# drprojects/superpoint_transformer

Measured on AMD Instinct MI355X. Metric: Mpoints/s SPT fwd+bwd on S3DIS-scale NAG, higher is better.
Workload: dtype f32 (the reference's shipped matmul class - configs/train.yaml:60-61 `float32_matmul_precision: high` = TF32 / bf16x3 next to `precision: 32` - as bf16x3: matrix products on the bf16 pipe with split operands, attention and the backward of the fused layers and of the attention blocks' Linears hi*hi +

## Files before the change

include/spt_hip.h:

```cpp
#ifndef SPT_HIP_H
#define SPT_HIP_H

#include <stddef.h>
#include <stdint.h>

#ifdef __cplusplus
extern "C" {
#endif

typedef void* spt_stream_t;

enum spt_reduce_op {
  SPT_SUM = 0,
  SPT_MEAN = 1,
  SPT_MIN = 2,
  SPT_MAX = 3
};

typedef struct spt_gn_fwd_tables {
  const float* weight;
  const float* mean_scale;
  float eps;
  float* mean;
  float* rstd;
// ... 347 lines not shown
size_t spt_relabel_consecutive_workspace_bytes(int64_t n_range);
int spt_relabel_consecutive(const int64_t* values, const int64_t* gather, int64_t k,
                            int64_t n_range, int64_t* new_values, int64_t* uniques,
                            int64_t* count, void* ws, size_t ws_bytes, spt_stream_t stream);

int spt_horizontal_edge_features_f32(
    const int64_t* se, int64_t e, int64_t n, const float* edge_attr7, const float* pos,
    const float* normal, const float* log_length, const float* log_surface,
    const float* log_volume, const float* log_size, int add_self_loops,
    int64_t* edge_index_out, float* edge_attr_out, spt_stream_t stream);
int spt_vertical_edge_features_f32(
    const int64_t* super_index, int64_t n, const float* child_pos, const float* child_normal,
    const float* child_log_length, const float* child_log_surface, const float* child_log_volume,
    const float* child_log_size, const float* parent_pos, const float* parent_normal,
    const float* parent_log_length, const float* parent_log_surface,
    const float* parent_log_volume, const float* parent_log_size, float* v_edge_attr,
    spt_stream_t stream);
int spt_edge_affinity_features_f32(const float* x, int64_t n, int C, const int64_t* edge_a,
                                   const int64_t* edge_b, int64_t e, float* out,
                                   spt_stream_t stream);
int spt_edge_affinity_features_bwd_f32(const float* x, const float* gout, int64_t n, int C,
                                       const int64_t* edge_a, const int64_t* edge_b, int64_t e,
                                       float* gend, spt_stream_t stream);

int spt_skinny_linear_supported(int K, int N);
int spt_skinny_linear_f32(const float* x, int64_t rows, int K, const float* W, const float* bias,
                          int N, float* y, spt_stream_t stream);
int spt_skinny_linear_wt_f32(const float* x, int64_t rows, int K, const float* Wt, int N, float* y,
                             spt_stream_t stream);
int spt_skinny_pre_supported(int K, int N, int num_graphs);
int spt_skinny_linear_pre_f32(const float* x, int64_t rows, int K, const float* W, const float* bias,
                              int N, float* y, const float* pre_am, const float* pre_scale,
                              const float* pre_bias, const int64_t* batch, int num_graphs,
                              const float* residual, spt_stream_t stream);
int spt_skinny_dw_pre_f32(const float* gy, const float* x, int64_t rows, int N, int K, float* gw,
                          float* gb, const float* pre_am, const float* pre_scale,
                          const float* pre_bias, const int64_t* batch, int num_graphs, void* ws,
                          size_t ws_bytes, spt_stream_t stream);
int spt_skinny_use_split_bf16(int mode);
int spt_skinny_linear_pre_m_f32(const float* x, int64_t rows, int K, const float* W, const float* bias,
                                int N, float* y, const float* pre_am, const float* pre_scale,
                                const float* pre_bias, const int64_t* batch, int num_graphs,
                                const float* residual, int mode, spt_stream_t stream);
int spt_skinny_linear_wt_m_f32(const float* x, int64_t rows, int K, const float* Wt, int N, float* y,
                               int mode, spt_stream_t stream);
int spt_skinny_dw_pre_m_f32(const float* gy, const float* x, int64_t rows, int N, int K, float* gw,
                            float* gb, const float* pre_am, const float* pre_scale,
                            const float* pre_bias, const int64_t* batch, int num_graphs, int mode,
                            void* ws, size_t ws_bytes, spt_stream_t stream);
int spt_skinny_dw_supported(int K, int N);
size_t spt_skinny_dw_workspace_bytes(int K, int N);
int spt_skinny_dw_f32(const float* gy, const float* x, int64_t rows, int N, int K, float* gw,
                      float* gb, void* ws, size_t ws_bytes, spt_stream_t stream);
int spt_narrow_linear_bwd_supported(int K, int N);
size_t spt_narrow_linear_bwd_workspace_bytes(int K, int N);
int spt_narrow_linear_bwd_f32(const float* gy, const float* x, const float* W, int64_t rows, int N,
                              int K, float* gx, float* gw, float* gb, void* ws, size_t ws_bytes,
                              spt_stream_t stream);

int spt_graphnorm_tables_f32(const double* total, int num_graphs, int d, const float* weight,
                             const float* mean_scale, float eps, float* mean, float* rstd,
                             float* am, float* scale, spt_stream_t stream);
int spt_graphnorm_apply_f32(const float* x, const int64_t* batch, int64_t r, int d,
                            int num_graphs, const float* am, const float* scale,
                            const float* bias, float act_slope, float* y, spt_stream_t stream);
int spt_graphnorm_bwd_stats_f32(const float* x, const float* gy, const int64_t* batch, int64_t r,
                                int d, int num_graphs, const float* am, const float* scale,
                                const float* bias, float act_slope, double* total, void* ws,
                                size_t ws_bytes, spt_stream_t stream);
size_t spt_graphnorm_bwd_stats_sparse_workspace_bytes(int64_t num_seg, int d, int num_graphs);
int spt_graphnorm_bwd_stats_sparse_f32(const float* x, const float* gout, const int32_t* arg,
                                       const int64_t* seg_graph, const int64_t* graph_rows,
                                       int64_t num_seg, int64_t n, int d, int num_graphs,
                                       const float* am, const float* scale, const float* bias,
                                       float act_slope, double* total, void* ws,
                                       size_t ws_bytes, spt_stream_t stream);
int spt_graphnorm_bwd_stats_sparse_ex_f32(
    const void* x, int x_is_bf16, const float* gout, const int32_t* arg, const int64_t* seg_graph,
    const int64_t* graph_rows, int64_t num_seg, int64_t n, int d, int num_graphs,
    const float* am, const float* scale, const float* bias, float act_slope, double* total,
    void* ws, size_t ws_bytes, spt_stream_t stream);
int spt_graphnorm_bwd_stats_sparse_raw_f32(
    const float* raw, const float* gout, const int32_t* arg, const int64_t* seg_graph,
    const int64_t* graph_rows, int64_t num_seg, int64_t n, int d, int num_graphs,
    const float* am, const float* scale, const float* bias, float act_slope, double* total,
    void* ws, size_t ws_bytes, spt_stream_t stream);
int spt_graphnorm_bwd_tables_f32(const double* total, int num_graphs, int d, const float* weight,
                                 const float* mean_scale, const float* mean, const float* rstd,
                                 float* c1, float* c2, float* c3, float* gweight, float* gbias,
                                 float* gmean_scale, spt_stream_t stream);

int spt_fused_linear_supported(int K, int N);
int spt_fused_linear_use_split_bf16(int mode);
size_t spt_fused_linear_workspace_bytes(int K, int N);
int spt_fused_linear_fwd_f32(const float* x, int64_t r0, int64_t r1, int K, const float* W,
                             int N, const float* pre_am, const float* pre_scale,
                             const float* pre_bias, float pre_slope, float* h, double* total,
                             void* ws, size_t ws_bytes, spt_stream_t stream);
int spt_fused_linear_bwd_f32(const float* gy, const float* h, int64_t r0, int64_t r1, int N,
                             const float* am, const float* scale, const float* bias,
                             float slope, const float* c1, const float* c2, const float* c3,
                             const float* xprev, int K, const float* pre_am,
                             const float* pre_scale, const float* pre_bias, float pre_slope,
                             const float* W, float* gx, float* gW, int accumulate,
                             double* prev_total, void* ws, size_t ws_bytes, spt_stream_t stream);
int spt_fused_linear_pooled_supported(int K, int N);
// ... 146 lines not shown
```

superpoint_transformer_amd/_lib.py:

```python
import ctypes
import os

import torch

_HERE = os.path.dirname(os.path.abspath(__file__))
LIB_PATH = os.path.join(_HERE, "lib", "libspt_hip.so")

_c = ctypes
_i64 = _c.c_int64
_int = _c.c_int
_p = _c.c_void_p
_sz = _c.c_size_t
_f32 = _c.c_float
_f64 = _c.c_double

SIGNATURES = {
    "spt_version": (_int, []),
    "spt_last_error": (_c.c_char_p, []),
    "spt_csr_build_workspace_bytes": (_sz, [_i64, _i64]),
    "spt_csr_build": (_int, [_p, _i64, _i64, _p, _p, _p, _sz, _p]),
    "spt_csr_pos_seg": (_int, [_p, _i64, _i64, _p, _p]),
    "spt_csr_gather_i64_i32": (_int, [_p, _p, _i64, _p, _p]),
    "spt_segcsr_reduce_f32": (_int, [_int, _p, _p, _p, _i64, _i64, _int, _p, _p, _p]),
    "spt_segcsr_max_affine_f32": (_int, [_p, _p, _p, _i64, _i64, _int, _p, _p, _p, _f32, _p, _p, _p, _p]),
# ... 132 lines not shown
                                                     _int, _p, _p, _p, _f32, _p, _p, _p, _p, _int, _p, _p,
                                                     _p, _f32, _p, _p, _p, _p, _p, _p, _int, _p, _sz, _p, _p]),
    "spt_csr_check_i64": (_int, [_p, _p, _p, _i64, _i64, _int, _p, _p]),
    "spt_csr_adopt_i64": (_int, [_p, _p, _p, _i64, _i64, _p, _p, _p, _p]),
    "spt_fused_linear_pool_supported": (_int, [_int, _int, _int]),
    "spt_fused_linear_pool_gram_len": (_sz, [_int]),
    "spt_fused_linear_pool_workspace_bytes": (_sz, [_int, _int]),
    "spt_fused_linear_fwd_pool_runs_f32": (_int, [_p, _p, _p, _p, _p, _i64, _i64, _int, _p, _p, _p, _int,
                                                  _int, _p, _int, _p, _p, _p, _f32, _f32, _p, _p, _p,
                                                  _f32, _p, _p, _p, _p, _p, _p, _p, _p, _p, _p, _int, _p,
                                                  _sz, _p]),
    "spt_fused_linear_bwd_pool_runs_f32": (_int, [_p, _p, _p, _p, _p, _p, _i64, _int, _p, _p, _p, _int,
                                                  _int, _p, _p, _p, _f32, _p, _p, _p, _p, _int, _p, _p,
                                                  _p, _f32, _p, _p, _p, _p, _p, _p, _int, _p, _sz, _p]),
    "spt_fused_linear_fwd_f32": (_int, [_p, _i64, _i64, _int, _p, _int, _p, _p, _p, _f32, _p, _p,
                                        _p, _sz, _p]),
    "spt_fused_linear_bwd_f32": (_int, [_p, _p, _i64, _i64, _int, _p, _p, _p, _f32, _p, _p, _p,
                                        _p, _int, _p, _p, _p, _f32, _p, _p, _p, _int, _p, _p,
                                        _sz, _p]),
    "spt_unit_sphere_norm_f32": (_int, [_p, _p, _p, _p, _p, _p, _i64, _i64, _p, _p, _p, _p]),
    "spt_unit_sphere_assemble_f32": (_int, [_p, _p, _p, _p, _p, _p, _i64, _i64, _p, _int, _p, _p, _p, _p]),
    "spt_unit_sphere_workspace_bytes": (_sz, [_i64, _i64]),
    "spt_unit_sphere_norm_ws_f32": (_int, [_p, _p, _p, _p, _p, _p, _i64, _i64, _p, _p, _p, _p, _sz, _p]),
    "spt_unit_sphere_assemble_ws_f32": (_int, [_p, _p, _p, _p, _p, _p, _i64, _i64, _p, _int, _p, _p, _p,
                                               _p, _sz, _p]),
    "spt_sparse_sample_workspace_bytes": (_sz, [_i64, _i64]),
    "spt_sparse_sample": (_int, [_p, _i64, _i64, _p, _int, _int, _c.c_uint64, _p, _p, _p, _sz, _p]),
    "spt_segment_std_f32": (_int, [_p, _p, _p, _i64, _int, _p, _p]),
    "spt_segment_mean_orientation_f32": (_int, [_p, _p, _p, _i64, _p, _p]),
    "spt_cluster_graph_edges_workspace_bytes": (_sz, [_i64, _int]),
    "spt_cluster_graph_edges": (_int, [_p, _p, _p, _i64, _int, _f32, _int, _p, _p, _p, _p, _sz, _p]),
    "spt_skinny_linear_supported": (_int, [_int, _int]),
    "spt_narrow_linear_bwd_supported": (_int, [_int, _int]),
    "spt_narrow_linear_bwd_workspace_bytes": (_sz, [_int, _int]),
    "spt_narrow_linear_bwd_f32": (_int, [_p, _p, _p, _i64, _int, _int, _p, _p, _p, _p, _sz, _p]),
    "spt_cross_entropy_workspace_bytes": (_sz, [_i64]),
    "spt_cross_entropy_fwd_f32": (_int, [_p, _p, _i64, _int, _i64, _p, _p, _p, _p, _sz, _p]),
    "spt_cross_entropy_bwd_f32": (_int, [_p, _p, _p, _i64, _int, _i64, _p, _p, _p, _p]),
    "spt_hist_loss_fwd_f32": (_int, [_p, _p, _i64, _int, _int, _int, _i64, _p, _p, _p, _p, _p, _sz, _p]),
    "spt_hist_loss_bwd_f32": (_int, [_p, _p, _i64, _int, _int, _int, _i64, _p, _p, _p, _p, _p]),
    "spt_confusion_matrix_i64": (_int, [_p, _p, _i64, _int, _int, _p, _p]),
    "spt_skinny_dw_supported": (_int, [_int, _int]),
    "spt_skinny_dw_workspace_bytes": (_sz, [_int, _int]),
    "spt_skinny_dw_f32": (_int, [_p, _p, _i64, _int, _int, _p, _p, _p, _sz, _p]),
    "spt_skinny_linear_f32": (_int, [_p, _i64, _int, _p, _p, _int, _p, _p]),
    "spt_skinny_linear_wt_f32": (_int, [_p, _i64, _int, _p, _int, _p, _p]),
    "spt_skinny_pre_supported": (_int, [_int, _int, _int]),
    "spt_skinny_linear_pre_f32": (_int, [_p, _i64, _int, _p, _p, _int, _p, _p, _p, _p, _p, _int, _p, _p]),
    "spt_skinny_dw_pre_f32": (_int, [_p, _p, _i64, _int, _int, _p, _p, _p, _p, _p, _p, _int, _p, _sz, _p]),
    "spt_skinny_use_split_bf16": (_int, [_int]),
    "spt_skinny_linear_pre_m_f32": (_int, [_p, _i64, _int, _p, _p, _int, _p, _p, _p, _p, _p, _int, _p, _int, _p]),
    "spt_skinny_linear_wt_m_f32": (_int, [_p, _i64, _int, _p, _int, _p, _int, _p]),
    "spt_skinny_dw_pre_m_f32": (_int, [_p, _p, _i64, _int, _int, _p, _p, _p, _p, _p, _p, _int, _int, _p, _sz, _p]),
    "spt_index_inverse": (_int, [_p, _i64, _i64, _p, _p]),
    "spt_select_edges_workspace_bytes": (_sz, [_i64]),
    "spt_select_edges": (_int, [_p, _i64, _i64, _p, _i64, _p, _i64, _p, _p, _p, _sz, _p]),
    "spt_cluster_select_workspace_bytes": (_sz, [_i64, _i64, _i64]),
    "spt_cluster_select": (_int, [_p, _p, _i64, _p, _i64, _i64, _p, _p, _p, _p, _p, _p, _sz, _p]),
    "spt_relabel_consecutive_workspace_bytes": (_sz, [_i64]),
    "spt_relabel_consecutive": (_int, [_p, _p, _i64, _i64, _p, _p, _p, _p, _sz, _p]),
    "spt_radius_ball_workspace_bytes": (_sz, [_i64]),
    "spt_radius_ball_f32": (_int, [_p, _i64, _p, _f32, _int, _p, _i64, _p, _p, _p, _sz, _p]),
    "spt_cluster_pair_anchors_f32": (_int, [_p, _p, _p, _p, _p, _i64, _i64, _int, _int, _p, _p, _p]),
    "spt_adjacency_stats_workspace_bytes": (_sz, [_i64]),
    "spt_adjacency_stats": (_int, [_p, _p, _i64, _i64, _int, _p, _p, _p, _sz, _p]),
    "spt_adjacency_regression": (_int, [_p, _p, _p, _i64, _i64, _int, _f32, _f32, _p, _p, _sz, _p]),
    "spt_adjacency_count_workspace_bytes": (_sz, [_i64]),
    "spt_adjacency_count": (_int, [_p, _i64, _i64, _int, _p, _p, _p, _i64, _int, _p, _p, _p, _sz, _p]),
    "spt_adjacency_fill_workspace_bytes": (_sz, [_i64, _i64]),
    "spt_adjacency_fill": (_int, [_p, _p, _i64, _i64, _int, _f32, _f32, _p, _p, _p, _p, _i64, _int, _int,
                                  _p, _p, _i64, _p, _p, _p, _p, _sz, _p]),
    "spt_ground_bounds_workspace_bytes": (_sz, [_i64]),
    "spt_ground_bounds_f32": (_int, [_p, _i64, _f32, _p, _p, _sz, _p]),
    "spt_ground_cell_min_f32": (_int, [_p, _i64, _f32, _i64, _i64, _i64, _i64, _p, _p]),
    "spt_ground_trim_workspace_bytes": (_sz, [_i64]),
    "spt_ground_trim_f32": (_int, [_p, _i64, _p, _int, _f32, _p, _f32, _p, _i64, _p, _i64, _p, _p, _sz, _p]),
    "spt_ground_ransac_workspace_bytes": (_sz, [_int]),
    "spt_ground_ransac_f32": (_int, [_p, _i64, _p, _p, _i64, _p, _p, _int, _f64, _p, _p, _p, _sz, _p]),
    "spt_ground_elevation_f32": (_int, [_p, _i64, _p, _f32, _p, _p]),
    "spt_point_color_workspace_bytes": (_sz, [_i64]),
    "spt_point_color_f32": (_int, [_p, _int, _i64, _int, _p, _i64, _p, _i64, _p, _i64, _p, _sz, _p]),
    "spt_point_density_f32": (_int, [_p, _i64, _p, _i64, _i64, _int, _p, _p]),
}


class GnFwdTables(ctypes.Structure):
    _fields_ = [("weight", _p), ("mean_scale", _p), ("eps", _f32), ("mean", _p), ("rstd", _p),
                ("am", _p), ("scale", _p)]


class GnBwdTables(ctypes.Structure):
    _fields_ = [("weight", _p), ("mean_scale", _p), ("mean", _p), ("rstd", _p), ("c1", _p), ("c2", _p),
                ("c3", _p), ("gweight", _p), ("gbias", _p), ("gmean_scale", _p)]


def _load():
    if not os.path.exists(LIB_PATH):
        raise ImportError(
            f"{LIB_PATH} is missing: run `python -c 'import __graft_entry__ as g; "
            f"g.build()'` (hipcc --offload-arch=gfx950). There is no fallback path.")
    lib = ctypes.CDLL(LIB_PATH)
    for name, (res, args) in SIGNATURES.items():
        fn = getattr(lib, name)
        fn.restype = res
        fn.argtypes = args
    return lib
# ... 29 lines not shown
```

superpoint_transformer_amd/csrc/skinny_linear.hip:

```cpp
#include "common.hpp"

namespace spt {
namespace skinny {

typedef float f32x4 __attribute__((ext_vector_type(4)));
constexpr int TR = 16;
constexpr int WAVES = 4;
constexpr int SLAB = 64;

typedef __bf16 bf16x8 __attribute__((ext_vector_type(8)));
typedef __bf16 bf16x4 __attribute__((ext_vector_type(4)));
typedef short s16x4 __attribute__((ext_vector_type(4)));

__host__ __device__ constexpr int skinny_planes(int PR) { return PR == 6 ? 3 : (PR == 3 ? 2 : 1); }
template <int NPL>
__device__ __forceinline__ void split_planes(const float (&x)[8], bf16x8 (&p)[NPL]) {
#pragma unroll
  for (int i = 0; i < 8; ++i) {
    const __bf16 a = (__bf16)x[i];
    p[0][i] = a;
    if constexpr (NPL >= 2) {
      const float r1 = x[i] - (float)a;
      const __bf16 b = (__bf16)r1;
      p[1][i] = b;
// ... 455 lines not shown
  }
  float* pw = partial + (size_t)wave * ((size_t)N * KF + N);
#pragma unroll
  for (int nb = 0; nb < 4; ++nb) {
    float v = bsum[nb];
    v += __shfl_xor(v, 16, 64);
    v += __shfl_xor(v, 32, 64);
    if (g == 0 && k0 == 0) pw[(size_t)N * KF + n0 + 16 * nb + c] = v;
  }
#pragma unroll
  for (int nb = 0; nb < 4; ++nb)
#pragma unroll
    for (int kb = 0; kb < KB; ++kb)
#pragma unroll
      for (int r = 0; r < 4; ++r)
        if (k0 + 16 * kb + c < KF)
          pw[(size_t)(n0 + 16 * nb + 4 * g + r) * KF + k0 + 16 * kb + c] = C[nb][kb][r];
}

__global__ __launch_bounds__(1024) void sum_tables_kernel(const float* __restrict__ partial, int ntab,
                                                          int len, int split, float* __restrict__ out0,
                                                          float* __restrict__ out1) {
  __shared__ float sl[64][17];
  const int cl = threadIdx.x & 15;
  const int col = blockIdx.x * 16 + cl;
  const int slice = threadIdx.x >> 4;
  float acc = 0.f;
  if (col < len) {
    const int per = (ntab + 63) / 64;
    const int lo = slice * per, hi = (lo + per < ntab) ? lo + per : ntab;
    int k = lo;
    for (; k + 16 <= hi; k += 16) {
      float a[16];
#pragma unroll
      for (int j = 0; j < 16; ++j) a[j] = partial[(size_t)(k + j) * len + col];
#pragma unroll
      for (int j = 0; j < 16; ++j) acc += a[j];
    }
    for (; k + 4 <= hi; k += 4) {
      const float a0 = partial[(size_t)k * len + col], a1 = partial[(size_t)(k + 1) * len + col];
      const float a2 = partial[(size_t)(k + 2) * len + col], a3 = partial[(size_t)(k + 3) * len + col];
      acc += a0; acc += a1; acc += a2; acc += a3;
    }
    for (; k < hi; ++k) acc += partial[(size_t)k * len + col];
  }
  sl[slice][cl] = acc;
  __syncthreads();
  if (slice == 0 && col < len) {
    float t = 0.f;
#pragma unroll
    for (int k = 0; k < 64; ++k) t += sl[k][cl];
    if (col < split) out0[col] = t;
    else if (out1) out1[col - split] = t;
  }
}

template <int NMAX>
__global__ __launch_bounds__(256) void narrow_linear_bwd_kernel(
    const float* __restrict__ gy, const float* __restrict__ x, const float* __restrict__ W,
    int64_t rows, int N, float* __restrict__ gx, float* __restrict__ partial, int K) {
  constexpr int RT = 16;
  const int lane = (threadIdx.x & 63) + 64 * blockIdx.y;
  const int64_t wave = (int64_t)blockIdx.x * (blockDim.x >> 6) + (threadIdx.x >> 6);
  const int64_t nwaves = (int64_t)gridDim.x * (blockDim.x >> 6);
  float w[NMAX], aw[NMAX], ab[NMAX];
#pragma unroll
  for (int n = 0; n < NMAX; ++n) {
    w[n] = (n < N) ? W[(size_t)n * K + lane] : 0.f;
    aw[n] = ab[n] = 0.f;
  }
  const int64_t nsteps = (rows + RT - 1) / RT;
  for (int64_t t = wave; t < nsteps; t += nwaves) {
    const int64_t row0 = t * RT;
    const int cnt = (int)((rows - row0) < RT ? (rows - row0) : RT);
    float gt[4];
    const int wl = threadIdx.x & 63;
#pragma unroll
    for (int q = 0; q < 4; ++q) {
      const int e = q * 64 + wl;
      gt[q] = (e < cnt * N) ? gy[row0 * N + e] : 0.f;
    }
    float xr[RT];
#pragma unroll
    for (int r = 0; r < RT; ++r) xr[r] = (r < cnt) ? x[(row0 + r) * K + lane] : 0.f;
    if (N == NMAX) {
#pragma unroll
      for (int r = 0; r < RT; ++r) {
        float dx = 0.f;
#pragma unroll
        for (int n = 0; n < NMAX; ++n) {
          const int e = r * NMAX + n;
          const float gv = __builtin_bit_cast(
              float, __builtin_amdgcn_readlane(__builtin_bit_cast(int, gt[e >> 6]), e & 63));
          dx = fmaf(gv, w[n], dx);
          aw[n] = fmaf(gv, xr[r], aw[n]);
          ab[n] += gv;
        }
        if (gx && r < cnt) gx[(row0 + r) * K + lane] = dx;
      }
    } else {
      for (int r = 0; r < cnt; ++r) {
        float dx = 0.f;
        for (int n = 0; n < N; ++n) {
          const int e = r * N + n;
          const float src = (e >> 6) == 0 ? gt[0] : ((e >> 6) == 1 ? gt[1] : ((e >> 6) == 2 ? gt[2] : gt[3]));
          const float gv = __shfl(src, e & 63, 64);
// ... 207 lines not shown
  }
  switch (K) {
#define SPT_SKINNY_PL(K4, PR_)                                                                     \
  skinny_linear_kernel<K4, 4, false, false, PR_><<<grid, WAVES * 64, 0, stream>>>(                 \
      x, rows, W, bias, N, y, nullptr, nullptr, nullptr, nullptr, 1, nullptr, ldwt);
#define SPT_SKINNY_PLS(K4)                                                                         \
  if (pr == 6) { SPT_SKINNY_PL(K4, 6) } else if (pr == 3) { SPT_SKINNY_PL(K4, 3) }                 \
  else if (pr == 1) { SPT_SKINNY_PL(K4, 1) } else { SPT_SKINNY_PL(K4, 0) }
    case 32:  SPT_SKINNY_PLS(8) break;
    case 64:  SPT_SKINNY_PLS(16) break;
#undef SPT_SKINNY_PLS
#undef SPT_SKINNY_PL
    case 128: skinny_linear_kernel<32><<<grid, WAVES * 64, 0, stream>>>(x, rows, W, bias, N, y, nullptr, nullptr, nullptr, nullptr, 1, nullptr, ldwt); break;
    case 256: {
      int64_t b4 = ceil_div(tiles, (int64_t)4);
      const int64_t cap4 = (int64_t)256 / slabs > 1 ? (int64_t)256 / slabs : 1;
      if (b4 > cap4) b4 = cap4;
      skinny_linear_wlds_kernel<64, 4><<<dim3((unsigned)b4, (unsigned)slabs), 4 * 64, 0, stream>>>(
          x, rows, W, bias, N, y, ldwt);
      break;
    }
    case 260: {
      int64_t b4 = ceil_div(tiles, (int64_t)4);
      const int64_t cap4 = (int64_t)256 / slabs > 1 ? (int64_t)256 / slabs : 1;
      if (b4 > cap4) b4 = cap4;
      skinny_linear_wlds_kernel<65, 4><<<dim3((unsigned)b4, (unsigned)slabs), 4 * 64, 0, stream>>>(
          x, rows, W, bias, N, y, ldwt);
      break;
    }
    default: {
      int64_t b8 = ceil_div(tiles, WAVES_L);
      const int64_t cap8 = (int64_t)256 * (K == 192 ? 2 : 1) / slabs > 1 ? (int64_t)256 * (K == 192 ? 2 : 1) / slabs : 1;
      if (b8 > cap8) b8 = cap8;
      if (K == 132)
        skinny_linear_wlds_kernel<33><<<dim3((unsigned)b8, (unsigned)slabs), WAVES_L * 64, 0, stream>>>(
            x, rows, W, bias, N, y, ldwt);
      else
      {
        const dim3 g8((unsigned)b8, (unsigned)slabs);
        if (pr >= 3)
          skinny_linear_wlds_kernel<48, WAVES_L, 3><<<g8, WAVES_L * 64, 0, stream>>>(x, rows, W, bias, N, y, ldwt);
        else if (pr == 1)
          skinny_linear_wlds_kernel<48, WAVES_L, 1><<<g8, WAVES_L * 64, 0, stream>>>(x, rows, W, bias, N, y, ldwt);
        else
          skinny_linear_wlds_kernel<48><<<g8, WAVES_L * 64, 0, stream>>>(x, rows, W, bias, N, y, ldwt);
      }
      break;
    }
  }
  SPT_CHECK_LAUNCH();
  return 0;
}

constexpr int NARROW_BLOCKS = 256;

extern "C" int spt_narrow_linear_bwd_supported(int K, int N) { return (K == 64 || K == 128) && N >= 1 && N <= 16; }
extern "C" size_t spt_narrow_linear_bwd_workspace_bytes(int K, int N) {
  return (size_t)NARROW_BLOCKS * 4 * (16 * K + 16) * sizeof(float);
}
extern "C" int spt_narrow_linear_bwd_f32(const float* gy, const float* x, const float* W,
                                         int64_t rows, int N, int K, float* gx, float* gw,
                                         float* gb, void* ws, size_t ws_bytes,
                                         spt_stream_t stream_) {
  hipStream_t stream = (hipStream_t)stream_;
  SPT_CHECK_ARG(rows >= 0, "bad shape");
  SPT_CHECK_ARG(spt_narrow_linear_bwd_supported(K, N), "(K, N) not built");
  SPT_CHECK_ARG(W && gw && (rows == 0 || (gy && x)), "null pointer");
  SPT_CHECK_ARG(ws && ws_bytes >= spt_narrow_linear_bwd_workspace_bytes(K, N), "workspace too small");
  if (rows == 0) {
    hipMemsetAsync(gw, 0, (size_t)N * K * sizeof(float), stream);
    if (gb) hipMemsetAsync(gb, 0, (size_t)N * sizeof(float), stream);
    return 0;
  }
  int64_t bx = ceil_div(ceil_div(rows, (int64_t)16), (int64_t)4);
  if (bx > NARROW_BLOCKS) bx = NARROW_BLOCKS;
  float* partial = (float*)ws;
  int nmax;
  if (N == 13) {
    nmax = 13;
    narrow_linear_bwd_kernel<13><<<dim3((unsigned)bx, K / 64), 256, 0, stream>>>(gy, x, W, rows, N, gx, partial, K);
  } else {
    nmax = 16;
    narrow_linear_bwd_kernel<16><<<dim3((unsigned)bx, K / 64), 256, 0, stream>>>(gy, x, W, rows, N, gx, partial, K);
  }
  (void)nmax;
  sum_tables_kernel<<<(N * (K + 1) + 15) / 16, 1024, 0, stream>>>(partial, (int)bx * 4, N * (K + 1), N * K,
                                                                  gw, gb);
  SPT_CHECK_LAUNCH();
  return 0;
}
```

superpoint_transformer_amd/ops.py:

```python
import contextlib
import ctypes
import os

import torch

from . import _lib
from . import precision as _precision
from .csr import EdgeCSR, SegmentCSR, csr_of, edge_csr_of

_OPS = {"sum": 0, "add": 0, "mean": 1, "min": 2, "max": 3}

_TIMERS = {}
_TIMER_PREFIXES = []
_TIMER_CAP = 8192


def enable_timer(name, prefix=False):
    _TIMERS[name] = []
    if prefix and name not in _TIMER_PREFIXES:
        _TIMER_PREFIXES.append(name)


def timer_count(name):
    return len(_TIMERS.get(name) or [])
# ... 804 lines not shown
    if (g.is_cuda and g.dtype == torch.float32 and weight.dtype == torch.float32 and g.dim() == 2
            and g.shape[0] >= _SKINNY_MIN_ROWS and n_in % 4 == 0 and n_in >= 64
            and _lib.lib.spt_skinny_linear_supported(n_out, n_in)):
        g = g.contiguous()
        w = weight.detach().contiguous()
        rows = g.shape[0]
        y = torch.empty((rows, n_in), dtype=torch.float32, device=g.device)
        with torch.cuda.device(g.device):
            st = _lib.lib.spt_skinny_linear_wt_m_f32(_lib.ptr(g), rows, n_out, _lib.ptr(w), n_in,
                                                     _lib.ptr(y), int(mode), _lib.stream_ptr(g.device))
        _lib.check(st, "spt_skinny_linear_wt_m_f32")
        return y
    wt = weight.detach().t().contiguous()
    return _skinny_launch(g, wt, None, mode) if _skinny_ok(g, wt) else g @ weight


def _dw_batched(g, x):
    n = x.shape[0]
    nb = n // _DW_CHUNK
    main = nb * _DW_CHUNK
    gw = None
    if nb > 0:
        gm = g[:main].view(nb, _DW_CHUNK, g.shape[1])
        xm = x[:main].view(nb, _DW_CHUNK, x.shape[1])
        gw = torch.bmm(gm.transpose(1, 2), xm).sum(0)
    if main < n:
        tail = g[main:].t() @ x[main:]
        gw = tail if gw is None else gw + tail
    return gw


def _skinny_dw_ok(g, x):
    return (x.is_cuda and x.dtype == torch.float32 and g.dtype == torch.float32
            and x.shape[0] >= _SKINNY_MIN_ROWS
            and _lib.lib.spt_skinny_dw_supported(x.shape[1], g.shape[1]))


def _skinny_dw(g, x, want_bias=False, mode=-1):
    g, x = g.contiguous(), x.detach().contiguous()
    rows, k = x.shape
    n = g.shape[1]
    gw = torch.empty((n, k), dtype=torch.float32, device=x.device)
    gb = torch.empty(n, dtype=torch.float32, device=x.device) if want_bias else None
    nb = _lib.lib.spt_skinny_dw_workspace_bytes(k, n)
    ws = _workspace(nb, x.device)
    with torch.cuda.device(x.device):
        st = _lib.lib.spt_skinny_dw_pre_m_f32(_lib.ptr(g), _lib.ptr(x), rows, n, k, _lib.ptr(gw),
                                              _lib.ptr(gb), None, None, None, None, 1, int(mode),
                                              _lib.ptr(ws), ws.numel(), _lib.stream_ptr(x.device))
    _lib.check(st, "spt_skinny_dw_pre_m_f32")
    return (gw, gb) if want_bias else gw


class _TallLinear(torch.autograd.Function):

    @staticmethod
    def forward(ctx, x, weight, bias):
        ctx.save_for_backward(x, weight)
        ctx.has_bias = bias is not None
        ctx.smode = _precision.skinny_mode()
        if _skinny_ok(x, weight):
            return _skinny_launch(x.detach(), weight.detach(), None if bias is None else bias.detach(),
                                  ctx.smode)
        return torch.nn.functional.linear(x, weight, bias)

    @staticmethod
    def backward(ctx, g):
        x, weight = ctx.saved_tensors
        g = g.contiguous()
        if (x.is_cuda and x.dtype == torch.float32 and g.dtype == torch.float32
                and weight.dtype == torch.float32 and x.shape[0] >= _SKINNY_MIN_ROWS
                and _lib.lib.spt_narrow_linear_bwd_supported(x.shape[1], g.shape[1])):
            xc, wc = x.detach().contiguous(), weight.detach().contiguous()
            rows, k = xc.shape
            n = g.shape[1]
            dev = xc.device
            gx = torch.empty_like(xc) if ctx.needs_input_grad[0] else None
            gw = torch.empty((n, k), dtype=torch.float32, device=dev)
            gb = torch.empty(n, dtype=torch.float32, device=dev) if ctx.has_bias else None
            nb = _lib.lib.spt_narrow_linear_bwd_workspace_bytes(k, n)
            ws = _workspace(nb, dev)
            with torch.cuda.device(dev):
                st = _lib.lib.spt_narrow_linear_bwd_f32(
                    _lib.ptr(g), _lib.ptr(xc), _lib.ptr(wc), rows, n, k, _lib.ptr(gx),
                    _lib.ptr(gw), _lib.ptr(gb), _lib.ptr(ws), ws.numel(), _lib.stream_ptr(dev))
            _lib.check(st, "spt_narrow_linear_bwd_f32")
            return gx, gw, gb
        gx = None
        smode = getattr(ctx, "smode", -1)
        if ctx.needs_input_grad[0]:
            gx = _input_grad(g, weight, smode)
        gw = gb = None
        want_gb = ctx.has_bias and ctx.needs_input_grad[2]
        if ctx.needs_input_grad[1]:
            if _skinny_dw_ok(g, x):
                gw = _skinny_dw(g, x, want_gb, smode)
                if want_gb:
                    gw, gb = gw
            else:
                gw = _dw_batched(g, x) if x.shape[0] >= 4 * _DW_CHUNK else g.t() @ x
        if want_gb and gb is None:
            gb = g.sum(0)
        return gx, gw, gb


def linear(x, weight, bias=None):
    if x.dim() != 2 or not x.is_cuda or x.shape[0] < _SKINNY_MIN_ROWS:
        return torch.nn.functional.linear(x, weight, bias)
    return _TallLinear.apply(x, weight, bias)


class _ResidualLinear(torch.autograd.Function):

    @staticmethod
    def forward(ctx, x, weight, bias, residual):
        ctx.save_for_backward(x, weight)
        ctx.has_bias = bias is not None
        ctx.smode = _precision.skinny_mode()
        xd, wd = x.detach().contiguous(), weight.detach().contiguous()
        rows, k = xd.shape
        n = wd.shape[0]
        y = torch.empty((rows, n), dtype=torch.float32, device=xd.device)
        with torch.cuda.device(xd.device):
            st = _lib.lib.spt_skinny_linear_pre_m_f32(
                _lib.ptr(xd), rows, k, _lib.ptr(wd),
                _lib.ptr(None if bias is None else bias.detach().contiguous()), n, _lib.ptr(y),
                None, None, None, None, 1, _lib.ptr(residual.detach().contiguous()),
                ctx.smode, _lib.stream_ptr(xd.device))
        _lib.check(st, "spt_skinny_linear_pre_m_f32")
        return y

    @staticmethod
    def backward(ctx, g):
        gx, gw, gb = _TallLinear.backward(ctx, g)
        return gx, gw, gb, g


_FUSE_PRENORM = os.environ.get("SPT_FUSE_PRENORM", "1") != "0"


def fuse_prenorm(on=None):
    global _FUSE_PRENORM
    prev = _FUSE_PRENORM
    if on is not None:
        _FUSE_PRENORM = bool(on)
    return prev
# ... 11 lines not shown
            and linear_residual_ok(residual, weight)):
        return _ResidualLinear.apply(x, weight, bias, residual)
    return residual + linear(x, weight, bias)


class _NormLinear(torch.autograd.Function):

    @staticmethod
    def forward(ctx, x, batch, num_graphs, gn_w, gn_b, gn_a, eps, weight, bias):
        _lib.require_cuda(x)
        xd = x.detach().contiguous()
        rows, d = xd.shape
        dev = xd.device
        B = int(num_graphs)
        if batch is not None:
            batch = batch.contiguous()
            if batch.dtype != torch.int64:
                batch = batch.long()
        w, b, a = (t.detach().float().contiguous() for t in (gn_w, gn_b, gn_a))
        wd = weight.detach().contiguous()
        bd = None if bias is None else bias.detach().contiguous()
        n = wd.shape[0]
        mean, rstd, am, sc = (torch.empty((B, d), dtype=torch.float32, device=dev) for _ in range(4))
        y = torch.empty((rows, n), dtype=torch.float32, device=dev)
        nb = _lib.lib.spt_graphnorm_workspace_bytes(rows, d, B)
        ws = _workspace(nb, dev)
        with torch.cuda.device(dev):
            st = _lib.lib.spt_graphnorm_stats_f32(
                _lib.ptr(xd), _lib.ptr(batch), rows, d, B, _lib.ptr(w), _lib.ptr(a), float(eps),
                _lib.ptr(mean), _lib.ptr(rstd), _lib.ptr(am), _lib.ptr(sc), _lib.ptr(ws),
                ws.numel(), _lib.stream_ptr(dev))
            _lib.check(st, "spt_graphnorm_stats_f32")
            smode = _precision.skinny_mode()
            st = _lib.lib.spt_skinny_linear_pre_m_f32(
                _lib.ptr(xd), rows, d, _lib.ptr(wd), _lib.ptr(bd), n, _lib.ptr(y), _lib.ptr(am),
                _lib.ptr(sc), _lib.ptr(b), _lib.ptr(batch), B, None, smode, _lib.stream_ptr(dev))
        _lib.check(st, "spt_skinny_linear_pre_m_f32")
        ctx.save_for_backward(xd, batch, w, b, a, mean, rstd, am, sc, wd)
        ctx.meta = (B, bias is not None)
        ctx.smode = smode
        ctx.set_materialize_grads(False)
        return y, x

    @staticmethod
    def backward(ctx, gy, gres):
        xd, batch, w, b, a, mean, rstd, am, sc, wd = ctx.saved_tensors
        B, has_bias = ctx.meta
        if gy is None:
            return gres, None, None, None, None, None, None, None, None
        rows, d = xd.shape
        n = wd.shape[0]
        dev = xd.device
        gy = gy.contiguous()
        gxn = _input_grad(gy, wd, ctx.smode)
        gw = torch.empty((n, d), dtype=torch.float32, device=dev)
        gb = torch.empty(n, dtype=torch.float32, device=dev) if has_bias else None
        ws = _workspace(_lib.lib.spt_skinny_dw_workspace_bytes(d, n), dev)
        with torch.cuda.device(dev):
            st = _lib.lib.spt_skinny_dw_pre_m_f32(
                _lib.ptr(gy), _lib.ptr(xd), rows, n, d, _lib.ptr(gw), _lib.ptr(gb), _lib.ptr(am),
                _lib.ptr(sc), _lib.ptr(b), _lib.ptr(batch), B, ctx.smode, _lib.ptr(ws), ws.numel(),
                _lib.stream_ptr(dev))
        _lib.check(st, "spt_skinny_dw_pre_m_f32")
        gx = torch.empty_like(xd)
        g_w, g_b, g_a = (torch.empty(d, dtype=torch.float32, device=dev) for _ in range(3))
        if gres is not None:
            gres = gres.contiguous()
        ws = _workspace(_lib.lib.spt_graphnorm_workspace_bytes(rows, d, B), dev)
        with torch.cuda.device(dev):
            st = _lib.lib.spt_graphnorm_bwd_acc_f32(
                _lib.ptr(xd), _lib.ptr(gxn), _lib.ptr(batch), rows, d, B, _lib.ptr(w), _lib.ptr(b),
                _lib.ptr(a), _lib.ptr(mean), _lib.ptr(rstd), 1.0, _lib.ptr(gres), _lib.ptr(gx),
                _lib.ptr(g_w), _lib.ptr(g_b), _lib.ptr(g_a), _lib.ptr(ws), ws.numel(),
                _lib.stream_ptr(dev))
        _lib.check(st, "spt_graphnorm_bwd_acc_f32")
        return gx, None, None, g_w, g_b, g_a, None, gw, gb


def norm_linear_ok(x, batch, num_graphs, weight):
    if not _FUSE_PRENORM or (batch is not None and num_graphs is None):
        return False
    B = 1 if batch is None else int(num_graphs)
    return bool(x.dim() == 2 and x.is_cuda and x.dtype == torch.float32
                and weight.dtype == torch.float32 and x.shape[0] >= _SKINNY_MIN_ROWS
                and _lib.lib.spt_skinny_pre_supported(x.shape[1], weight.shape[0], B)
                and _lib.lib.spt_skinny_dw_supported(x.shape[1], weight.shape[0]))


_BCHK_ATTR = "_spt_batch_checked"


def _check_batch_ids(batch, B):
    if batch is None or _host_ptr(batch, B) is not None:
        return
    key = (batch._version, int(B), batch.data_ptr(), batch.numel())
    if getattr(batch, _BCHK_ATTR, None) == key:
        return
    if batch.numel():
        lo, hi = torch.aminmax(batch)
        if int(lo) < 0 or int(hi) >= int(B):
            raise ValueError(f"graph ids of `batch` must lie in [0, {int(B)}): found [{int(lo)}, {int(hi)}]")
    try:
        setattr(batch, _BCHK_ATTR, key)
    except Exception:
        pass


def norm_linear(x, batch, num_graphs, gn_weight, gn_bias, gn_mean_scale, eps, weight, bias):
    B = 1 if batch is None else int(num_graphs)
    _check_batch_ids(batch, B)
    return _NormLinear.apply(x, batch, B, gn_weight, gn_bias, gn_mean_scale, float(eps), weight, bias)


class _CrossEntropy(torch.autograd.Function):
    @staticmethod
    def forward(ctx, logits, target, ignore_index):
# ... 811 lines not shown
```

Baseline: 375.8.

## Fuse skinny linear backward input-grad and weight-grad into one bf16-split MFMA kernel

Measured after the change: 382.3, median of 6. 1.7% higher.

```diff
diff --git a/include/spt_hip.h b/include/spt_hip.h
--- a/include/spt_hip.h
+++ b/include/spt_hip.h
@@ -423,6 +423,14 @@
 size_t spt_skinny_dw_workspace_bytes(int K, int N);
 int spt_skinny_dw_f32(const float* gy, const float* x, int64_t rows, int N, int K, float* gw,
                       float* gb, void* ws, size_t ws_bytes, spt_stream_t stream);
+int spt_skinny_linear_bwd_supported(int K, int N, int num_graphs, int mode);
+size_t spt_skinny_linear_bwd_workspace_bytes(int K, int N);
+int spt_skinny_linear_bwd_m_f32(const float* gy, const float* x, const float* W, int64_t rows, int N,
+                                int K, float* gx, float* gw, float* gb, const float* pre_am,
+                                const float* pre_scale, const float* pre_bias, const int64_t* batch,
+                                int num_graphs, int mode, void* ws, size_t ws_bytes,
+                                spt_stream_t stream);
+int spt_skinny_bwd_fused(int on);
 int spt_narrow_linear_bwd_supported(int K, int N);
 size_t spt_narrow_linear_bwd_workspace_bytes(int K, int N);
 int spt_narrow_linear_bwd_f32(const float* gy, const float* x, const float* W, int64_t rows, int N,
diff --git a/superpoint_transformer_amd/_lib.py b/superpoint_transformer_amd/_lib.py
--- a/superpoint_transformer_amd/_lib.py
+++ b/superpoint_transformer_amd/_lib.py
@@ -208,6 +208,11 @@
     "spt_skinny_linear_pre_m_f32": (_int, [_p, _i64, _int, _p, _p, _int, _p, _p, _p, _p, _p, _int, _p, _int, _p]),
     "spt_skinny_linear_wt_m_f32": (_int, [_p, _i64, _int, _p, _int, _p, _int, _p]),
     "spt_skinny_dw_pre_m_f32": (_int, [_p, _p, _i64, _int, _int, _p, _p, _p, _p, _p, _p, _int, _int, _p, _sz, _p]),
+    "spt_skinny_linear_bwd_supported": (_int, [_int, _int, _int, _int]),
+    "spt_skinny_linear_bwd_workspace_bytes": (_sz, [_int, _int]),
+    "spt_skinny_linear_bwd_m_f32": (_int, [_p, _p, _p, _i64, _int, _int, _p, _p, _p, _p, _p, _p, _p, _int, _int,
+                                           _p, _sz, _p]),
+    "spt_skinny_bwd_fused": (_int, [_int]),
     "spt_index_inverse": (_int, [_p, _i64, _i64, _p, _p]),
     "spt_select_edges_workspace_bytes": (_sz, [_i64]),
     "spt_select_edges": (_int, [_p, _i64, _i64, _p, _i64, _p, _i64, _p, _p, _p, _sz, _p]),
diff --git a/superpoint_transformer_amd/csrc/skinny_linear.hip b/superpoint_transformer_amd/csrc/skinny_linear.hip
--- a/superpoint_transformer_amd/csrc/skinny_linear.hip
+++ b/superpoint_transformer_amd/csrc/skinny_linear.hip
@@ -531,6 +531,197 @@
     for (int k = 0; k < 64; ++k) t += sl[k][cl];
     if (col < split) out0[col] = t;
     else if (out1) out1[col - split] = t;
+  }
+}
+
+constexpr int BF_ROWS = 64;
+constexpr int BF_WAVES = 8;
+constexpr int BF_BLOCKS = 256;
+__host__ __device__ constexpr int bf_per_cu(int NN) { return NN == 64 ? 2 : 1; }
+typedef __attribute__((address_space(3))) bf16x4 lds_bf16x4;
+__device__ __forceinline__ bf16x8 read_tr_operand(const __bf16* at, int ld) {
+  const bf16x4 a = __builtin_amdgcn_ds_read_tr16_b64_v4bf16((lds_bf16x4*)at);
+  const bf16x4 b = __builtin_amdgcn_ds_read_tr16_b64_v4bf16((lds_bf16x4*)(at + 16 * ld));
+  return __builtin_shufflevector(a, b, 0, 1, 2, 3, 4, 5, 6, 7);
+}
+template <int NPL>
+__device__ __forceinline__ void split_planes4(const float4& v, bf16x4 (&p)[NPL]) {
+  const float x[4] = {v.x, v.y, v.z, v.w};
+#pragma unroll
+  for (int i = 0; i < 4; ++i) {
+    const __bf16 a = (__bf16)x[i];
+    p[0][i] = a;
+    if constexpr (NPL >= 2) p[1][i] = (__bf16)(x[i] - (float)a);
+  }
+}
+template <int NN, bool PRE, int PR>
+__global__ __launch_bounds__(BF_WAVES * 64, 2 * bf_per_cu(NN)) void skinny_bwd_fused_kernel(
+    const float* __restrict__ gy, const float* __restrict__ x, const float* __restrict__ W, int64_t rows,
+    float* __restrict__ gx, float* __restrict__ partial, const float* __restrict__ pam,
+    const float* __restrict__ psc, const float* __restrict__ pbs, const int64_t* __restrict__ batch,
+    int PB) {
+  constexpr int K = 64, NT = BF_WAVES * 64, LDG = NN + 16, LDX = K + 16, LDW = NN + 8;
+  constexpr int NPL = skinny_planes(PR), KS = NN / 32, NBW = NN / 64;
+  constexpr int VG = BF_ROWS * NN / 4 / NT, VX = BF_ROWS * K / 4 / NT;
+  static_assert(NN % 64 == 0 && (PR == 1 || PR == 3), "whole 64-column slabs, a bf16 mode");
+  static_assert(BF_ROWS * NN / 4 % NT == 0 && BF_ROWS * K / 4 % NT == 0, "whole float4 rounds");
+  constexpr int GPL = NPL == 1 ? 2 : NPL;
+  static_assert(GPL * BF_ROWS * LDG * 2 >= BF_ROWS * NN * 4, "the gb slots fit the gy planes");
+  __shared__ __attribute__((aligned(16))) __bf16 g_pl[GPL * BF_ROWS * LDG];
+  __shared__ __attribute__((aligned(16))) __bf16 x_pl[NPL * BF_ROWS * LDX];
+  __shared__ __attribute__((aligned(16))) __bf16 w_pl[NPL * K * LDW];
+  __shared__ __attribute__((aligned(16))) float ptab[PRE ? 2 * PRE_MAX + K : 4];
+  const int tid = threadIdx.x;
+  const int lane = tid & 63;
+  const int wid = __builtin_amdgcn_readfirstlane(tid >> 6);
+  const int g = lane >> 4, c = lane & 15;
+
+  for (int q = tid; q < K * (NN / 8); q += NT) {
+    const int k = q & (K - 1), n8 = q / K;
+    float wv[8];
+#pragma unroll
+    for (int j = 0; j < 8; ++j) wv[j] = W[(size_t)(8 * n8 + j) * K + k];
+    bf16x8 pl[NPL];
+    split_planes<NPL>(wv, pl);
+#pragma unroll
+    for (int p = 0; p < NPL; ++p) *reinterpret_cast<bf16x8*>(w_pl + p * K * LDW + k * LDW + 8 * n8) = pl[p];
+  }
+  if constexpr (PRE) {
+    for (int i = tid; i < PB * K; i += NT) {
+      ptab[i] = pam[i];
+      ptab[PRE_MAX + i] = psc[i];
+    }
+    for (int i = tid; i < K; i += NT) ptab[2 * PRE_MAX + i] = pbs[i];
+  }
+
+  const int rt = wid >> 1, nh = wid & 1;
+  const int kp = wid & 1, nb0 = (wid >> 1) * NBW;
+  f32x4 CW[NBW][2];
+#pragma unroll
+  for (int i = 0; i < NBW; ++i) CW[i][0] = CW[i][1] = (f32x4){0.f, 0.f, 0.f, 0.f};
+  float4 bs[VG];
+#pragma unroll
+  for (int v = 0; v < VG; ++v) bs[v] = make_float4(0.f, 0.f, 0.f, 0.f);
+
+  const int64_t ntiles = (rows + BF_ROWS - 1) / BF_ROWS;
+  float4 ng[VG], nx[VX];
+  int xg[VX];
+  auto fetch = [&](int64_t t) {
+    const int64_t gbase = t * BF_ROWS * (int64_t)NN, glim = rows * (int64_t)NN;
+#pragma unroll
+    for (int v = 0; v < VG; ++v) {
+      const int64_t e = gbase + (int64_t)(v * NT + tid) * 4;
+      ng[v] = (e < glim) ? *reinterpret_cast<const float4*>(gy + e) : make_float4(0.f, 0.f, 0.f, 0.f);
+    }
+#pragma unroll
+    for (int v = 0; v < VX; ++v) {
+      const int q = v * NT + tid;
+      const int64_t row = t * BF_ROWS + q / (K / 4);
+      nx[v] = (row < rows) ? *reinterpret_cast<const float4*>(x + row * K + (q & (K / 4 - 1)) * 4)
+                           : make_float4(0.f, 0.f, 0.f, 0.f);
+      if constexpr (PRE) xg[v] = (row < rows) ? (batch ? (int)batch[row] : 0) : -1;
+    }
+  };
+  if ((int64_t)blockIdx.x < ntiles) fetch(blockIdx.x);
+  for (int64_t t = blockIdx.x; t < ntiles; t += gridDim.x) {
+    __syncthreads();
+#pragma unroll
+    for (int v = 0; v < VG; ++v) {
+      const int q4 = (v * NT + tid) * 4, rr = q4 / NN, col = q4 - rr * NN;
+      bs[v].x += ng[v].x; bs[v].y += ng[v].y; bs[v].z += ng[v].z; bs[v].w += ng[v].w;
+      bf16x4 pl[NPL];
+      split_planes4<NPL>(ng[v], pl);
+#pragma unroll
+      for (int p = 0; p < NPL; ++p) *reinterpret_cast<bf16x4*>(g_pl + p * BF_ROWS * LDG + rr * LDG + col) = pl[p];
+    }
+#pragma unroll
+    for (int v = 0; v < VX; ++v) {
+      const int q = v * NT + tid, rr = q / (K / 4), ch = q & (K / 4 - 1);
+      float4 w = nx[v];
+      if constexpr (PRE) {
+        if (xg[v] >= 0) {
+          const float4 a = *reinterpret_cast<const float4*>(ptab + xg[v] * K + ch * 4);
+          const float4 sc4 = *reinterpret_cast<const float4*>(ptab + PRE_MAX + xg[v] * K + ch * 4);
+          const float4 b4 = *reinterpret_cast<const float4*>(ptab + 2 * PRE_MAX + ch * 4);
+          w.x = fmaf(w.x - a.x, sc4.x, b4.x); w.y = fmaf(w.y - a.y, sc4.y, b4.y);
+          w.z = fmaf(w.z - a.z, sc4.z, b4.z); w.w = fmaf(w.w - a.w, sc4.w, b4.w);
+        }
+      }
+      bf16x4 pl[NPL];
+      split_planes4<NPL>(w, pl);
+#pragma unroll
+      for (int p = 0; p < NPL; ++p) *reinterpret_cast<bf16x4*>(x_pl + p * BF_ROWS * LDX + rr * LDX + ch * 4) = pl[p];
+    }
+    __syncthreads();
+    if (t + gridDim.x < ntiles) fetch(t + gridDim.x);
+
+    {
+      f32x4 C[2] = {(f32x4){0.f, 0.f, 0.f, 0.f}, (f32x4){0.f, 0.f, 0.f, 0.f}};
+      const __bf16* al = g_pl + (16 * rt + c) * LDG + 8 * g;
+#pragma unroll
+      for (int ks = 0; ks < KS; ++ks) {
+        bf16x8 Ap[NPL];
+#pragma unroll
+        for (int p = 0; p < NPL; ++p) Ap[p] = *reinterpret_cast<const bf16x8*>(al + p * BF_ROWS * LDG + 32 * ks);
+#pragma unroll
+        for (int i = 0; i < 2; ++i) {
+          bf16x8 Bp[NPL];
+#pragma unroll
+          for (int p = 0; p < NPL; ++p)
+            Bp[p] = *reinterpret_cast<const bf16x8*>(w_pl + p * K * LDW + (16 * (2 * nh + i) + c) * LDW +
+                                                     32 * ks + 8 * g);
+          C[i] = mfma_planes<PR>(Ap, Bp, C[i]);
+        }
+      }
+#pragma unroll
+      for (int r = 0; r < 4; ++r) {
+        const int64_t row = t * BF_ROWS + 16 * rt + 4 * g + r;
+        if (row < rows) {
+#pragma unroll
+          for (int i = 0; i < 2; ++i)
+            __builtin_nontemporal_store(C[i][r], gx + row * K + 16 * (2 * nh + i) + c);
+        }
+      }
+    }
+
+#pragma unroll
+    for (int s = 0; s < BF_ROWS / 32; ++s) {
+      const int r0 = 32 * s + 4 * g + ((lane >> 2) & 3), c0 = 4 * (lane & 3);
+      bf16x8 Ap[NBW][NPL];
+#pragma unroll
+      for (int i = 0; i < NBW; ++i)
+#pragma unroll
+        for (int p = 0; p < NPL; ++p)
+          Ap[i][p] = read_tr_operand(g_pl + p * BF_ROWS * LDG + r0 * LDG + 16 * (nb0 + i) + c0, LDG);
+#pragma unroll
+      for (int kk = 0; kk < 2; ++kk) {
+        bf16x8 Bp[NPL];
+#pragma unroll
+        for (int p = 0; p < NPL; ++p)
+          Bp[p] = read_tr_operand(x_pl + p * BF_ROWS * LDX + r0 * LDX + 16 * (2 * kp + kk) + c0, LDX);
+#pragma unroll
+        for (int i = 0; i < NBW; ++i) CW[i][kk] = mfma_planes<PR>(Ap[i], Bp, CW[i][kk]);
+      }
+    }
+  }
+
+  float* pw = partial + (size_t)blockIdx.x * ((size_t)NN * K + NN);
+#pragma unroll
+  for (int i = 0; i < NBW; ++i)
+#pragma unroll
+    for (int kk = 0; kk < 2; ++kk)
+#pragma unroll
+      for (int r = 0; r < 4; ++r)
+        pw[(size_t)(16 * (nb0 + i) + 4 * g + r) * K + 16 * (2 * kp + kk) + c] = CW[i][kk][r];
+  __syncthreads();
+  float* slots = reinterpret_cast<float*>(g_pl);
+#pragma unroll
+  for (int v = 0; v < VG; ++v) *reinterpret_cast<float4*>(slots + (v * NT + tid) * 4) = bs[v];
+  __syncthreads();
+  if (tid < NN) {
+    float v = 0.f;
+    for (int rr = 0; rr < BF_ROWS; ++rr) v += slots[rr * NN + tid];
+    pw[(size_t)NN * K + tid] = v;
   }
 }
 
@@ -844,6 +1035,57 @@
   return 0;
 }
 
+static std::atomic<int> g_bwd_fused{[] { const char* e = getenv("SPT_SKINNY_BWD_FUSED"); return (e && atoi(e) == 0) ? 0 : 1; }()};
+extern "C" int spt_skinny_bwd_fused(int on) {
+  const int prev = g_bwd_fused;
+  if (on >= 0) g_bwd_fused = on ? 1 : 0;
+  return prev;
+}
+extern "C" int spt_skinny_linear_bwd_supported(int K, int N, int num_graphs, int mode) {
+  return K == 64 && (N == 64 || N == 192) && skinny_pr_bwd(mode) != 0 && num_graphs >= 1 &&
+         num_graphs * K <= PRE_MAX;
+}
+extern "C" size_t spt_skinny_linear_bwd_workspace_bytes(int K, int N) {
+  return (size_t)BF_BLOCKS * bf_per_cu(N) * N * (K + 1) * sizeof(float);
+}
+extern "C" int spt_skinny_linear_bwd_m_f32(const float* gy, const float* x, const float* W, int64_t rows,
+                                           int N, int K, float* gx, float* gw, float* gb,
+                                           const float* pre_am, const float* pre_scale,
+                                           const float* pre_bias, const int64_t* batch, int num_graphs,
+                                           int mode, void* ws, size_t ws_bytes, spt_stream_t stream_) {
+  const int pr = skinny_pr_bwd(mode);
+  hipStream_t stream = (hipStream_t)stream_;
+  SPT_CHECK_ARG(rows >= 0, "bad shape");
+  const bool pre = pre_am != nullptr;
+  SPT_CHECK_ARG(spt_skinny_linear_bwd_supported(K, N, pre ? num_graphs : 1, mode),
+                "(K, N) not built, the f32-exact mode or num_graphs * K too large");
+  SPT_CHECK_ARG(!pre || (pre_scale && pre_bias), "pre-normalisation: incomplete tables");
+  SPT_CHECK_ARG(gw && (rows == 0 || (gy && x && W && gx)), "null pointer");
+  SPT_CHECK_ARG(ws && ws_bytes >= spt_skinny_linear_bwd_workspace_bytes(K, N), "workspace too small");
+  if (rows == 0) {
+    hipMemsetAsync(gw, 0, (size_t)N * K * sizeof(float), stream);
+    if (gb) hipMemsetAsync(gb, 0, (size_t)N * sizeof(float), stream);
+    return 0;
+  }
+  int64_t bx = ceil_div(rows, (int64_t)BF_ROWS);
+  if (bx > BF_BLOCKS * bf_per_cu(N)) bx = BF_BLOCKS * bf_per_cu(N);
+  float* partial = (float*)ws;
+#define SPT_BF(NN_, PRE_, PR_)                                                                      \
+  skinny_bwd_fused_kernel<NN_, PRE_, PR_><<<(unsigned)bx, BF_WAVES * 64, 0, stream>>>(               \
+      gy, x, W, rows, gx, partial, pre_am, pre_scale, pre_bias, batch, num_graphs);
+#define SPT_BFS(NN_, PRE_) if (pr == 3) { SPT_BF(NN_, PRE_, 3) } else { SPT_BF(NN_, PRE_, 1) }
+  if (N == 192) {
+    if (pre) { SPT_BFS(192, true) } else { SPT_BFS(192, false) }
+  } else {
+    if (pre) { SPT_BFS(64, true) } else { SPT_BFS(64, false) }
+  }
+#undef SPT_BFS
+#undef SPT_BF
+  sum_tables_kernel<<<(N * (K + 1) + 15) / 16, 1024, 0, stream>>>(partial, (int)bx, N * (K + 1), N * K, gw, gb);
+  SPT_CHECK_LAUNCH();
+  return 0;
+}
+
 constexpr int NARROW_BLOCKS = 256;
 
 extern "C" int spt_narrow_linear_bwd_supported(int K, int N) { return (K == 64 || K == 128) && N >= 1 && N <= 16; }
diff --git a/superpoint_transformer_amd/ops.py b/superpoint_transformer_amd/ops.py
--- a/superpoint_transformer_amd/ops.py
+++ b/superpoint_transformer_amd/ops.py
@@ -880,6 +880,45 @@
     return (gw, gb) if want_bias else gw
 
 
+_BWD_ROUTE = {"fused": 0, "split": 0}
+
+
+def skinny_bwd_fused(on=None):
+    return bool(_lib.lib.spt_skinny_bwd_fused(-1 if on is None else int(bool(on))))
+
+
+def skinny_bwd_route_counts():
+    return dict(_BWD_ROUTE)
+
+
+def _skinny_bwd_ok(g, x, weight, num_graphs, mode):
+    return bool(x.is_cuda and x.dtype == torch.float32 and g.dtype == torch.float32
+                and weight.dtype == torch.float32 and x.dim() == 2 and x.shape[0] >= _SKINNY_MIN_ROWS
+                and _lib.lib.spt_skinny_bwd_fused(-1)
+                and _lib.lib.spt_skinny_linear_bwd_supported(x.shape[1], g.shape[1], int(num_graphs),
+                                                             int(mode)))
+
+
+def _skinny_bwd(g, x, weight, want_bias, mode, pre=None):
+    g, x, w = g.contiguous(), x.detach().contiguous(), weight.detach().contiguous()
+    rows, k = x.shape
+    n = g.shape[1]
+    dev = x.device
+    gx = torch.empty((rows, k), dtype=torch.float32, device=dev)
+    gw = torch.empty((n, k), dtype=torch.float32, device=dev)
+    gb = torch.empty(n, dtype=torch.float32, device=dev) if want_bias else None
+    am, sc, pb, batch, B = pre if pre is not None else (None, None, None, None, 1)
+    ws = _workspace(_lib.lib.spt_skinny_linear_bwd_workspace_bytes(k, n), dev)
+    with torch.cuda.device(dev):
+        st = _lib.lib.spt_skinny_linear_bwd_m_f32(
+            _lib.ptr(g), _lib.ptr(x), _lib.ptr(w), rows, n, k, _lib.ptr(gx), _lib.ptr(gw), _lib.ptr(gb),
+            _lib.ptr(am), _lib.ptr(sc), _lib.ptr(pb), _lib.ptr(batch), int(B), int(mode), _lib.ptr(ws),
+            ws.numel(), _lib.stream_ptr(dev))
+    _lib.check(st, "spt_skinny_linear_bwd_m_f32")
+    _BWD_ROUTE["fused"] += 1
+    return gx, gw, gb
+
+
 class _TallLinear(torch.autograd.Function):
 
     @staticmethod
@@ -916,10 +955,13 @@
             return gx, gw, gb
         gx = None
         smode = getattr(ctx, "smode", -1)
+        want_gb = ctx.has_bias and ctx.needs_input_grad[2]
+        if ctx.needs_input_grad[0] and ctx.needs_input_grad[1] and _skinny_bwd_ok(g, x, weight, 1, smode):
+            return _skinny_bwd(g, x, weight, want_gb, smode)
+        _BWD_ROUTE["split"] += 1
         if ctx.needs_input_grad[0]:
             gx = _input_grad(g, weight, smode)
         gw = gb = None
-        want_gb = ctx.has_bias and ctx.needs_input_grad[2]
         if ctx.needs_input_grad[1]:
             if _skinny_dw_ok(g, x):
                 gw = _skinny_dw(g, x, want_gb, smode)
@@ -1037,16 +1079,20 @@
         n = wd.shape[0]
         dev = xd.device
         gy = gy.contiguous()
-        gxn = _input_grad(gy, wd, ctx.smode)
-        gw = torch.empty((n, d), dtype=torch.float32, device=dev)
-        gb = torch.empty(n, dtype=torch.float32, device=dev) if has_bias else None
-        ws = _workspace(_lib.lib.spt_skinny_dw_workspace_bytes(d, n), dev)
-        with torch.cuda.device(dev):
-            st = _lib.lib.spt_skinny_dw_pre_m_f32(
-                _lib.ptr(gy), _lib.ptr(xd), rows, n, d, _lib.ptr(gw), _lib.ptr(gb), _lib.ptr(am),
-                _lib.ptr(sc), _lib.ptr(b), _lib.ptr(batch), B, ctx.smode, _lib.ptr(ws), ws.numel(),
-                _lib.stream_ptr(dev))
-        _lib.check(st, "spt_skinny_dw_pre_m_f32")
+        if ctx.needs_input_grad[7] and _skinny_bwd_ok(gy, xd, wd, B, ctx.smode):
+            gxn, gw, gb = _skinny_bwd(gy, xd, wd, has_bias, ctx.smode, (am, sc, b, batch, B))
+        else:
+            _BWD_ROUTE["split"] += 1
+            gxn = _input_grad(gy, wd, ctx.smode)
+            gw = torch.empty((n, d), dtype=torch.float32, device=dev)
+            gb = torch.empty(n, dtype=torch.float32, device=dev) if has_bias else None
+            ws = _workspace(_lib.lib.spt_skinny_dw_workspace_bytes(d, n), dev)
+            with torch.cuda.device(dev):
+                st = _lib.lib.spt_skinny_dw_pre_m_f32(
+                    _lib.ptr(gy), _lib.ptr(xd), rows, n, d, _lib.ptr(gw), _lib.ptr(gb), _lib.ptr(am),
+                    _lib.ptr(sc), _lib.ptr(b), _lib.ptr(batch), B, ctx.smode, _lib.ptr(ws), ws.numel(),
+                    _lib.stream_ptr(dev))
+            _lib.check(st, "spt_skinny_dw_pre_m_f32")
         gx = torch.empty_like(xd)
         g_w, g_b, g_a = (torch.empty(d, dtype=torch.float32, device=dev) for _ in range(3))
         if gres is not None:
```
